# thodson-usgs/discontinuum

Hardware: AMD Instinct MI355X
Metric: GP fits/sec (NLL+grad step) at n=8192 d=3, 1/2/4/8 MI355X (higher is better)
Workload: dtype f64

## Files before the change

discontinuum_amd/_lib.py:

```python
from __future__ import annotations

import ctypes as C
import os

_HERE = os.path.dirname(os.path.abspath(__file__))
LIB_PATH = os.path.join(_HERE, "libdgp_hip.so")

F64, F32 = 0, 1
MODEL_LOADEST, MODEL_RATING = 0, 1
OUT_NLL, OUT_QUAD, OUT_LOGDET, OUT_INFO, OUT_DTHETA, OUT_SUM_DR, OUT_DR_W0, OUT_SUM_DNOISE, OUT_LEN = 0, 1, 2, 3, 4, 28, 29, 31, 32
BUF_XT, BUF_A, BUF_T, BUF_S, BUF_Z, BUF_ALPHA = range(6)
BUF_INFO, BUF_SCAL = 6, 7
OPT_LAUUM64_MAX_TILES, OPT_SYRK_SLOTS, OPT_TRTRI_SMALL, OPT_REFINE, OPT_SYRK_ORDER, OPT_LAUUM_ORDER, OPT_CHAIN_YIELD, OPT_FUSED_GRAD, OPT_GROUP_GEMM = range(9)
OPT_POTRF_SCHEDULE, OPT_POTRF_SWEEP, OPT_POTRF_SOLVE, OPT_POTRF_OVERLAP, OPT_POTRF_SLOTS, OPT_POTRF_TAIL, OPT_POTRF_TAIL_SWEEP = range(9, 16)
TIME_GRAM, TIME_POTRF, TIME_SYRK_SUM, TIME_SYRK_N, TIME_TRTRI, TIME_LAUUM, TIME_SOLVE, TIME_GRAD, TIME_SYRK_FLOP, TIME_COUNT = range(10)


E_ARG, E_MODEL, E_WORKSPACE, E_STATE, E_FULL, E_NOCONV = -1, -2, -3, -4, -5, -6


class DGPLibraryError(RuntimeError):
    pass


class DGPError(RuntimeError):
    def __init__(self, code, where, msg):
        super().__init__(f"{where} failed with code {code}: {msg}")
        self.code = code


_vp, _i, _i64, _sz = C.c_void_p, C.c_int, C.c_int64, C.c_size_t
_dp = C.POINTER(C.c_double)

SIGNATURES = {
    "dgp_version": (_i, []),
    "dgp_last_error": (C.c_char_p, []),
    "dgp_model_ntheta": (_i, [_i, _i]),
# ... 124 lines not shown
```

discontinuum_amd/csrc/dgp_api.hip:

```cpp
#include <mutex>
#include <new>
#include <stdio.h>
#include <stdlib.h>
#include <string.h>
#include <utility>
#include <vector>

#include "../../include/dgp_hip.h"
#include "dgp_common.h"
#include "dgp_internal.h"

using namespace dgp;

static thread_local char g_err[256] = "";
static int fail(int code, const char* msg) {
  snprintf(g_err, sizeof(g_err), "%s", msg);
  return code;
}
static int hipfail(hipError_t e, const char* where) {
  snprintf(g_err, sizeof(g_err), "%s: %s", where, hipGetErrorString(e));
  return (int)e;
}

struct PinnedRing {
// ... 30 lines not shown
      if (have_ev[i]) (void)hipEventDestroy(ev[i]);
      if (buf[i]) (void)hipHostFree(buf[i]);
    }
  }
};

struct dgp_plan {
  int model, dtype, d, ntheta;
  PinnedRing ring;
  int* nsite_host;
  int B;
  size_t site_bytes;
  void* pre;
  void* pre2;
  int pre_ready;
  Tuning tune;
  int refine;
  int* nsite;
  const void* dr_w;
  int64_t n, N;
  size_t elem;
  char* ws;
  size_t ws_bytes;
  void *Xt, *A, *Tm, *S, *z, *alpha, *gpart, *spart, *scal, *snap;
  int* info;
  hipStream_t sc;
  int lookahead, early;
  int have_inputs, have_factor, have_inverse;
  hipStream_t s2, s3;
  hipEvent_t xev[8];
  int have_xev;
  hipEvent_t* ev;
  int nev;
  int timing, n_syrk, timed_valid;
  double syrk_flop;
  hipEvent_t* tev;
  hipEvent_t* sev;
  int nsev;
};
enum { TS_GRAM = 0, TS_POTRF, TS_TRTRI, TS_LAUUM, TS_SOLVE, TS_GRAD, TS_COUNT };

static size_t align_up(size_t x) { return (x + 255) & ~(size_t)255; }

struct Layout {
  size_t Xt, A, Tm, S, z, alpha, gpart, spart, scal, info, snap, total;
};
static Layout layout(const dgp_plan* p) {
  Layout L;
  const size_t e = p->elem, N = (size_t)p->N;
  size_t o = 0;
  L.Xt = o; o += align_up(e * N * p->d);
  L.A = o; o += align_up(e * N * N);
  L.Tm = o; o += align_up(e * N * N);
  L.S = o; o += align_up(e * N * N);
  L.z = o; o += align_up(e * N);
  L.alpha = o; o += align_up(e * N);
  L.gpart = o; o += align_up(e * (size_t)gram_grad_partials(p->N));
  L.spart = o; o += align_up(e * (size_t)solve_partials(p->N));
  L.scal = o; o += align_up(e * 16);
  L.info = o; o += align_up(sizeof(int) * POTRF_INFO_INTS);
  L.snap = o; o += align_up(e * 2 * DGP_TILE_HOST * DGP_TILE_HOST);
  L.total = o;
  return L;
}

static int default_lookahead() { return 2; }
static int group_size(int lookahead, int batch, long nbk) {
  if (!lookahead) return 0;
  if (const char* e = getenv("DGP_GROUP")) return atoi(e) < 2 ? 2 : atoi(e);
  if (batch >= 4) return 4;
  return nbk >= 256 ? 8 : (nbk >= 96 ? 4 : 2);
}

#define EARLY_WG_CAP 384
#define EARLY_RESERVED_CUS 64

extern "C" {

int dgp_version(void) { return 1; }
const char* dgp_last_error(void) { return g_err; }
int dgp_model_ntheta(int model, int d) { return model_ntheta(model, d); }
int dgp_composite_define(const int* spec, int nspec, int* model_out) {
  if (!spec || nspec < 2 || !model_out) return fail(DGP_E_ARG, "dgp_composite_define: null argument");
  const int id = composite_define(spec, nspec);
// ... 89 lines not shown
  return 0;
}

int dgp_plan_set_workspace(dgp_plan* p, void* dev_ptr, size_t bytes) {
  if (!p || !dev_ptr) return fail(DGP_E_ARG, "dgp_plan_set_workspace: null");
  const Layout L = layout(p);
  if (bytes < dgp_plan_workspace_bytes(p))
    return fail(DGP_E_WORKSPACE, "dgp_plan_set_workspace: workspace too small");
  p->site_bytes = L.total;
  if (((uintptr_t)dev_ptr & 255) != 0) return fail(DGP_E_ARG, "dgp_plan_set_workspace: pointer must be 256-byte aligned");
  p->ws = (char*)dev_ptr;
  p->ws_bytes = bytes;
  p->Xt = p->ws + L.Xt;
  p->A = p->ws + L.A;
  p->Tm = p->ws + L.Tm;
  p->S = p->ws + L.S;
  p->z = p->ws + L.z;
  p->alpha = p->ws + L.alpha;
  p->gpart = p->ws + L.gpart;
  p->spart = p->ws + L.spart;
  p->scal = p->ws + L.scal;
  p->info = (int*)(p->ws + L.info);
  p->snap = p->ws + L.snap;
  p->pre = pre_scratch_bytes(p->B) ? (void*)(p->ws + L.total * (size_t)p->B) : nullptr;
  p->pre2 = p->pre ? (void*)((char*)p->pre + align_up(pre_scratch_bytes(p->B))) : nullptr;
  p->nsite = nullptr;
  p->dr_w = nullptr;
  if (p->B > 1) {
    p->nsite = (int*)(p->ws + L.total * (size_t)p->B + 2 * align_up(pre_scratch_bytes(p->B)));
    delete[] p->nsite_host;
    p->nsite_host = new (std::nothrow) int[(size_t)p->B];
    if (!p->nsite_host) return fail(DGP_E_ARG, "dgp_plan_set_workspace: out of host memory");
    for (int b = 0; b < p->B; ++b) p->nsite_host[b] = (int)p->n;
    hipError_t e = hipMemcpy(p->nsite, p->nsite_host, sizeof(int) * (size_t)p->B, hipMemcpyHostToDevice);
    if (e != hipSuccess) return hipfail(e, "dgp_plan_set_workspace: hipMemcpy");
  }
  p->have_inputs = p->have_factor = 0;
  return 0;
}

int dgp_plan_set_option(dgp_plan* p, int key, int64_t value) {
  if (!p) return fail(DGP_E_ARG, "dgp_plan_set_option: null plan");
  switch (key) {
    case DGP_OPT_LAUUM64_MAX_TILES:
      if (value < 0 || value > (1 << 30)) return fail(DGP_E_ARG, "dgp_plan_set_option: value out of range");
      p->tune.lauum64_max_tiles = (int)value;
// ... 20 lines not shown
    case DGP_OPT_GROUP_GEMM:
      p->tune.group_gemm = value ? 1 : 0;
      return 0;
    case DGP_OPT_POTRF_SCHEDULE:
      if (value < 0 || value > 1) return fail(DGP_E_ARG, "dgp_plan_set_option: value out of range");
      p->tune.potrf_schedule = (int)value;
      return 0;
    case DGP_OPT_POTRF_SWEEP:
    case DGP_OPT_POTRF_TAIL:
    case DGP_OPT_POTRF_TAIL_SWEEP:
      if (value < 0 || value > (1 << 20)) return fail(DGP_E_ARG, "dgp_plan_set_option: value out of range");
      (key == DGP_OPT_POTRF_SWEEP ? p->tune.potrf_sweep : key == DGP_OPT_POTRF_TAIL ? p->tune.potrf_tail : p->tune.potrf_tail_sweep) = (int)value;
      return 0;
    case DGP_OPT_POTRF_SOLVE:
      p->tune.potrf_solve = value ? 1 : 0;
      return 0;
    case DGP_OPT_POTRF_OVERLAP:
      p->tune.potrf_overlap = value ? 1 : 0;
      return 0;
    case DGP_OPT_POTRF_SLOTS:
      if (value < 1 || value > (1 << 20)) return fail(DGP_E_ARG, "dgp_plan_set_option: value out of range");
      p->tune.potrf_slots = (int)value;
      return 0;
    case DGP_OPT_REFINE:
      if (p->dtype != DGP_F32 && value) return fail(DGP_E_ARG, "dgp_plan_set_option: refinement applies to float32 plans");
      p->refine = value ? 1 : 0;
      return 0;
    default:
      return fail(DGP_E_ARG, "dgp_plan_set_option: unknown option");
  }
}
int dgp_plan_get_option(const dgp_plan* p, int key, int64_t* value) {
  if (!p || !value) return fail(DGP_E_ARG, "dgp_plan_get_option: null argument");
  switch (key) {
    case DGP_OPT_LAUUM64_MAX_TILES: *value = p->tune.lauum64_max_tiles; return 0;
    case DGP_OPT_SYRK_SLOTS: *value = p->tune.syrk_slots; return 0;
    case DGP_OPT_TRTRI_SMALL: *value = p->tune.trtri_small; return 0;
    case DGP_OPT_REFINE: *value = p->refine; return 0;
    case DGP_OPT_SYRK_ORDER: *value = p->tune.syrk_super; return 0;
    case DGP_OPT_LAUUM_ORDER: *value = p->tune.lauum_super; return 0;
    case DGP_OPT_CHAIN_YIELD: *value = p->tune.chain_yield; return 0;
    case DGP_OPT_FUSED_GRAD: *value = p->tune.fused_grad; return 0;
    case DGP_OPT_GROUP_GEMM: *value = p->tune.group_gemm; return 0;
    case DGP_OPT_POTRF_SCHEDULE:
      *value = p->tune.potrf_schedule < 0 ? (p->B >= 4 ? potrf_schedule_auto(p->B, p->N / DGP_TILE_HOST, p->elem) : 0) : p->tune.potrf_schedule;
      return 0;
    case DGP_OPT_POTRF_SWEEP: *value = p->tune.potrf_sweep; return 0;
    case DGP_OPT_POTRF_SOLVE: *value = p->tune.potrf_solve; return 0;
    case DGP_OPT_POTRF_OVERLAP: *value = p->tune.potrf_overlap; return 0;
    case DGP_OPT_POTRF_SLOTS: *value = p->tune.potrf_slots; return 0;
    case DGP_OPT_POTRF_TAIL: *value = p->tune.potrf_tail; return 0;
    case DGP_OPT_POTRF_TAIL_SWEEP: *value = p->tune.potrf_tail_sweep; return 0;
    default: return fail(DGP_E_ARG, "dgp_plan_get_option: unknown option");
  }
}

int dgp_plan_set_lookahead(dgp_plan* p, int level) {
  if (!p) return fail(DGP_E_ARG, "null plan");
  p->lookahead = level ? default_lookahead() : 0;
  p->early = level >= 2 && !getenv("DGP_NO_EARLY_TRTRI");
  return 0;
}

size_t dgp_plan_site_stride_bytes(const dgp_plan* p) { return p ? layout(p).total : 0; }

int dgp_plan_buffer(const dgp_plan* p, int which, void** dev_ptr, int64_t* ld) {
  if (!p || !dev_ptr || !p->ws) return fail(DGP_E_ARG, "dgp_plan_buffer: null / no workspace");
  void* q = nullptr;
  switch (which) {
    case DGP_BUF_XT: q = p->Xt; break;
    case DGP_BUF_A: q = p->A; break;
    case DGP_BUF_T: q = p->Tm; break;
    case DGP_BUF_S: q = p->S; break;
    case DGP_BUF_Z: q = p->z; break;
    case DGP_BUF_ALPHA: q = p->alpha; break;
// ... 268 lines not shown
    const long N = p->N;
    const size_t nb = (size_t)(N / 64), part_bytes = nb * nb * 64 * sizeof(double);
    if (gram_residual_scratch_bytes(N) > (size_t)N * N * sizeof(float)) return 0;
    char* base = (char*)p->S;
    double* part = (double*)base;
    double* rho64 = (double*)(base + part_bytes);
    float* rho32 = (float*)(base + part_bytes + (size_t)N * sizeof(double));
    float* delta = rho32 + N;
    const Batch bt = batch_of<float>(p);
    const long ps = bt.ws / 2;
    void* staging = p->pre2 ? p->ring.acquire(pre_scratch_bytes(p->B)) : nullptr;
    int rc = gram_residual<float>(p->model, p->d, (const float*)p->Xt, N, (int)p->n, theta, (const float*)noise, (const float*)r,
                                  (const float*)p->alpha, part, rho64, rho32, s, bt, ps, bt.ws, p->pre2, staging);
    if (staging) p->ring.commit(s);
    if (rc) return rc;
    return refine_solve<float>((const float*)p->Tm, N, (const float*)r, (int)p->n, rho64, rho32, (float*)p->z, delta,
                               (float*)p->alpha, (float*)p->spart, (float*)p->scal + 1, s, bt, ps, bt.ws);
  }
}

template <typename T>
static int run_grad(dgp_plan* p, const double* theta, void* dtheta, hipStream_t s) {
  return gram_grad<T>(p->model, p->d, (const T*)p->Xt, p->N, (int)p->n, theta, (const T*)p->S, (const T*)p->alpha,
                      (T*)p->gpart, (T*)dtheta, s, batch_of<T>(p), DGP_OUT_LEN, p->pre, p->pre_ready != 0);
}

template <typename T>
static bool solve_overlap(const dgp_plan* p) {
  if (p->N < 1024 || p->N > 6144 || !p->lookahead || !p->ev || p->nev < 2 || !p->s2) return false;
  return !(sizeof(T) == 4 && p->refine);
}

template <typename T>
static int fit_step(dgp_plan* p, const double* theta, const void* r, const void* noise, void* out, void* dr,
                    void* dnoise, int with_grad, hipStream_t s) {
  int rc;
  if ((rc = ensure_timing(p))) return rc;
  tick(p, TS_GRAM, 0, s);
  if ((rc = run_gram<T>(p, theta, noise, s))) return rc;
  tick(p, TS_GRAM, 1, s);
  if ((rc = ensure_async(p, s)) || (rc = ensure_early(p, s))) return rc;
  tick(p, TS_POTRF, 0, s);
  const int nbk = (int)(p->N / DGP_TILE_HOST);
  const bool early = early_applies(p) && p->s3 != nullptr;
  const Batch bt = batch_of<T>(p);
  if (early) {
    struct Early {
// ... 1164 lines not shown
```

discontinuum_amd/csrc/dgp_chol.hip:

```cpp
#include <stdlib.h>
#include <string.h>
#include <algorithm>
#include <mutex>
#include "dgp_diag.h"
#include "dgp_gemm.h"
#include "dgp_gemm_dma.h"
#include "dgp_internal.h"
#include "dgp_schedule.h"

namespace dgp {

static constexpr int NB = DGP_TILE;
static constexpr int SMID_TABLE = 4096;
template <typename T>
struct Prefetch {
  static constexpr bool F64 = sizeof(T) == 8;
  static constexpr int LAUUM = F64 ? 2 : 4, TRTRI = F64 ? 1 : 4, SYRK = F64 ? 1 : 2;
};

#define DGP_INFO_CHAIN_TIMEOUT (-7)
#define CHAIN_WAIT_TICKS 200000000LL
__device__ __forceinline__ bool chain_reached(const int* word, int value) {
  return __hip_atomic_load(word, __ATOMIC_RELAXED, __HIP_MEMORY_SCOPE_AGENT) >= value;
}
// ... 101 lines not shown
  if (super > 0) super_decode(nfull + sub / split, nt, super, bi, bj);
  else tri_decode(nfull + sub / split, bi, bj);
  syrk_cut_tile<T>(A, ld, k, nk, (long)(bi + jbeg) * NB, (long)(bj + jbeg) * NB, split, sub % split, smem);
}

const Tuning& default_tuning() {
  static const Tuning t = [] {
    Tuning v;
    v.lauum64_max_tiles = getenv("DGP_LAUUM64") ? atoi(getenv("DGP_LAUUM64")) : 1000;
    v.syrk_slots = getenv("DGP_SYRK_SLOTS") ? atoi(getenv("DGP_SYRK_SLOTS")) : 512;
    v.trtri_small = getenv("DGP_TRTRI_SMALL") ? atol(getenv("DGP_TRTRI_SMALL")) : 1024;
    v.syrk_super = getenv("DGP_SYRK_ORDER") ? atoi(getenv("DGP_SYRK_ORDER")) : 0;
    v.lauum_super = getenv("DGP_LAUUM_ORDER") ? atoi(getenv("DGP_LAUUM_ORDER")) : 0;
    v.chain_yield = getenv("DGP_CHAIN_YIELD") ? atoi(getenv("DGP_CHAIN_YIELD")) : 1;
    v.fused_grad = getenv("DGP_FUSED_GRAD") ? atoi(getenv("DGP_FUSED_GRAD")) : 0;
    v.group_gemm = getenv("DGP_GROUP_GEMM") ? atoi(getenv("DGP_GROUP_GEMM")) : 0;
    v.potrf_schedule = getenv("DGP_POTRF_SCHEDULE") ? (atoi(getenv("DGP_POTRF_SCHEDULE")) != 0 ? 1 : 0) : -1;
    v.potrf_sweep = getenv("DGP_POTRF_SWEEP") ? std::max(0, atoi(getenv("DGP_POTRF_SWEEP"))) : 0;
    v.potrf_tail = getenv("DGP_POTRF_TAIL") ? std::max(0, atoi(getenv("DGP_POTRF_TAIL"))) : 0;
    v.potrf_tail_sweep = getenv("DGP_POTRF_TAIL_SWEEP") ? std::max(0, atoi(getenv("DGP_POTRF_TAIL_SWEEP"))) : 0;
    v.potrf_solve = getenv("DGP_POTRF_SOLVE") ? atoi(getenv("DGP_POTRF_SOLVE")) : 0;
    v.potrf_overlap = getenv("DGP_POTRF_OVERLAP") ? atoi(getenv("DGP_POTRF_OVERLAP")) : 0;
    v.potrf_slots = getenv("DGP_POTRF_SLOTS") ? std::max(1, atoi(getenv("DGP_POTRF_SLOTS"))) : 768;
    if (v.syrk_slots < 1) v.syrk_slots = 1;
    return v;
  }();
  return t;
}
int potrf_schedule_auto(int B, long nbk, int elem) { return (elem == 8 && B >= 32 && nbk > 4) ? 1 : 0; }
struct SyrkShape {
  int nfull, split;
  unsigned grid;
  explicit SyrkShape(int ntiles, int slots = 512) {
    if (slots < 1) slots = 1;
    const double cost[5] = {0, 1.0, 0.55, 0, 0.30};
    const int whole = ntiles / slots * slots, rem = ntiles - whole;
    nfull = ntiles;
    split = 1;
    double best = (ntiles + slots - 1) / slots * cost[1];
    for (int g = 2; g <= 4; g += 2) {
      const double c = whole / slots * cost[1] + (g * rem + slots - 1) / slots * cost[g];
      if (rem > 0 && c < best - 1e-9) {
        best = c;
        nfull = whole;
        split = g;
      }
// ... 1153 lines not shown
```

discontinuum_amd/csrc/dgp_gram.hip:

```cpp
#include <mutex>
#include <string.h>
#include "dgp_internal.h"
#include "dgp_models.h"
#include "dgp_gram_shared.h"

namespace dgp {

size_t pre_scratch_bytes(int B) { return B > DGP_MAX_BATCH ? (size_t)B * DGP_PRE_SLOT_BYTES : 0; }

#define DGP_C_MAXMODELS 64
static CompositeDesc g_comp[DGP_C_MAXMODELS];
static int g_ncomp = 0;
static std::mutex g_comp_mtx;
static thread_local const CompositeDesc* g_comp_cur = nullptr;
const CompositeDesc* composite_current() { return g_comp_cur; }
static const CompositeDesc* composite_get(int model) {
  const int slot = model - DGP_MODEL_COMPOSITE_BASE;
  return (slot >= 0 && slot < g_ncomp) ? &g_comp[slot] : nullptr;
}
bool composite_select(int model, int d) {
  g_comp_cur = composite_get(model);
  return g_comp_cur && g_comp_cur->d == d;
}

// ... 27 lines not shown
      fc.ls = (signed char)th;
      th += ard ? ndims : 1;
      fc.period = type == DGP_FAC_PERIODIC ? (signed char)th++ : (signed char)-1;
      if (th > DGP_MAX_THETA) return -2;
    }
  }
  if (i != nspec) return -2;
  c.ntheta = (unsigned char)th;
  std::lock_guard<std::mutex> lock(g_comp_mtx);
  for (int k = 0; k < g_ncomp; ++k)
    if (memcmp(&g_comp[k], &c, sizeof(c)) == 0) return DGP_MODEL_COMPOSITE_BASE + k;
  if (g_ncomp >= DGP_C_MAXMODELS) return -5;
  g_comp[g_ncomp] = c;
  return DGP_MODEL_COMPOSITE_BASE + g_ncomp++;
}

int model_ntheta(int model, int d) {
  if (model == DGP_MODEL_LOADEST) return (d >= 2 && d <= 6) ? 2 * d + 5 : -1;
  if (model == DGP_MODEL_RATING) return d == 2 ? 16 : -1;
  if (const CompositeDesc* c = composite_get(model)) return c->d == d ? c->ntheta : -1;
  return -1;
}

int model_nterms(int model, int d) {
  if (model == DGP_MODEL_LOADEST) return (d >= 2 && d <= 6) ? 3 : -1;
  if (model == DGP_MODEL_RATING) return d == 2 ? 5 : -1;
  if (const CompositeDesc* c = composite_get(model)) return c->d == d ? c->nterms : -1;
  return -1;
}

int model_input_differentiable(int model, int d, int col) {
  if (model_ntheta(model, d) < 0 || col < 0 || col >= d) return -1;
  const CompositeDesc* c = composite_get(model);
  if (!c) return 1;
  for (int t = 0; t < c->nterms; ++t)
    for (int f = 0; f < c->term[t].nfac; ++f) {
      const CompositeDesc::Fac& fc = c->term[t].fac[f];
      if (fc.type != DGP_FAC_MATERN || fc.nu2 != 1) continue;
      for (int j = 0; j < fc.ndims; ++j)
        if (fc.dims[j] == col) return 0;
    }
  return 1;
}

template <typename T>
__global__ __launch_bounds__(256) void pack_x_kernel(const T* __restrict__ X, int n, int d, long N, T* __restrict__ Xt,
// ... 93 lines not shown
      if (gi >= n || gj >= m) v = T(0);
      out[b] = v;
    }
    store4<T>(Ks + gi * Mp + (long)bj * 64 + tx * 4, out);
  }
}

template <typename T, typename M>
__global__ __launch_bounds__(256) void gram_diag_kernel(const T* __restrict__ Xst, long Mp, int m, const PreBatch<M> pb,
                                                        T* __restrict__ kss, long wbs) {
  const typename M::Pre& pre = pb.get();
  Xst = site(Xst, wbs);
  kss = site(kss, wbs);
  exp_table_init<T>();
  __syncthreads();
  const long j = (long)blockIdx.x * 256 + threadIdx.x;
  if (j >= Mp) return;
  T x[M::NX], f[M::NF], dummy[M::NTHETA];
#pragma unroll
  for (int c = 0; c < M::NX; ++c) x[c] = Xst[(long)c * Mp + j];
  M::features(x, pre, f);
  T v = M::template pair<false>(f, f, pre, T(0), dummy);
  kss[j] = j < m ? v : T(0);
}

template <typename T, typename M, int MODE>
__global__ __launch_bounds__(256) void gram_grad_kernel(const T* __restrict__ Xt, long N, int n, const PreBatch<M> pb,
                                                        const T* __restrict__ S, const T* __restrict__ alpha,
                                                        const T* __restrict__ beta, T* __restrict__ partials, long bs,
                                                        const int* __restrict__ ns, long wbs ) {
  n = site_n(ns, n);
  const typename M::Pre& pre = pb.get();
  Xt = site(Xt, bs);
  if (MODE == 0) S = site(S, bs);
  alpha = site(alpha, bs);
  partials = site(partials, MODE == 0 ? bs : wbs);
  if (MODE == 1) beta = site(beta, wbs);
  __shared__ T sfi[M::NF][64], sfj[M::NF][64], sai[64], saj[64], sbi[64], sbj[64];
  __shared__ T red[4][M::NTHETA];
  int bi, bj;
  tri_decode(blockIdx.x, bi, bj);
  const int t = threadIdx.x;
  exp_table_init<T>();
  if (t < 64) {
    stage_strip<T, M>(Xt, N, (long)bi * 64, pre, sfi, t);
    sai[t] = alpha[(long)bi * 64 + t];
// ... 311 lines not shown
  const int nb = (int)(N / 64);
  const double* p = part + (i / 64) * (long)nb * 64 + (i & 63);
  double s0 = 0.0, s1 = 0.0, s2 = 0.0, s3 = 0.0;
  int b = 0;
  for (; b + 4 <= nb; b += 4) {
    s0 += p[(long)b * 64];
    s1 += p[(long)(b + 1) * 64];
    s2 += p[(long)(b + 2) * 64];
    s3 += p[(long)(b + 3) * 64];
  }
  for (; b < nb; ++b) s0 += p[(long)b * 64];
  double v = 0.0;
  if (i < n) v = (double)r[i] - (double)noise[i] * (double)alpha[i] - ((s0 + s1) + (s2 + s3));
  rho64[i] = v;
  rho32[i] = (TS)v;
}

template <typename T>
int pack_x(const T* X, int n, int d, long N, T* Xt, hipStream_t s, Batch bt) {
  pack_x_kernel<T><<<dim3((unsigned)((N + 255) / 256), 1, (unsigned)bt.B), dim3(256), 0, s>>>(X, n, d, N, Xt, bt.ws, bt.ns);
  return (int)hipGetLastError();
}

template <typename T>
int gram_sym(int model, int d, const T* Xt, long N, int n, const double* theta, const T* noise, T* K, hipStream_t s,
             Batch bt, void* pre_scratch, void* pre_staging, long k_stride, long noise_stride, bool pre_ready) {
  const int nt = model_ntheta(model, d);
  if (nt < 0) return -2;
  const long nb = N / 64;
  const unsigned grid = (unsigned)(nb * (nb + 1) / 2);
  const long ks = k_stride >= 0 ? k_stride : bt.ws, nstr = noise_stride >= 0 ? noise_stride : (long)n;
  DGP_DISPATCH_MODEL(model, d, (gram_sym_kernel<T, M><<<dim3(grid, 1, (unsigned)bt.B), dim3(256), 0, s>>>(
                                   Xt, N, n, prepare_batch<M>(theta, nt, bt.B, pre_scratch, !pre_ready, s, pre_staging), noise, K, bt.ws, bt.ns,
                                   ks, nstr)));
  return (int)hipGetLastError();
}

template <typename T>
int gram_sym_panel(int model, int d, const T* Xt, long N, int n, const double* theta, const T* noise, T* K, long row0, long row1,
                   hipStream_t s, Batch bt, void* pre_scratch, long k_stride, long noise_stride) {
  const int nt = model_ntheta(model, d);
  if (nt < 0) return -2;
  const long b0 = row0 / 64, b1 = row1 / 64;
  const long t0 = b0 * (b0 + 1) / 2, t1 = b1 * (b1 + 1) / 2;
  DGP_DISPATCH_MODEL(model, d, (gram_sym_kernel<T, M, true><<<dim3((unsigned)(t1 - t0), 1, (unsigned)bt.B), dim3(256), 0, s>>>(
                                   Xt, N, n, prepare_batch<M>(theta, nt, bt.B, pre_scratch, false, s), noise, K, bt.ws, bt.ns, k_stride,
// ... 11 lines not shown
                                   Xt, N, n, Xst, Mp, m, prepare_batch<M>(theta, nt, bt.B, pre_scratch, true, s, pre_staging), Ks, bt.ws,
                                   wbs, bt.ns)));
  return (int)hipGetLastError();
}

template <typename T>
int gram_diag(int model, int d, const T* Xst, long Mp, int m, const double* theta, T* kss, hipStream_t s, Batch bt, long wbs,
              void* pre_scratch) {
  const int nt = model_ntheta(model, d);
  if (nt < 0) return -2;
  dim3 grid((unsigned)((Mp + 255) / 256), 1, (unsigned)bt.B);
  DGP_DISPATCH_MODEL(model, d, (gram_diag_kernel<T, M><<<grid, dim3(256), 0, s>>>(
                                   Xst, Mp, m, prepare_batch<M>(theta, nt, bt.B, pre_scratch, false, s), kss, wbs)));
  return (int)hipGetLastError();
}

long gram_grad_partials(long N) {
  const long nb = N / 64;
  return nb * (nb + 1) / 2 * DGP_MAX_THETA;
}

template <typename T>
int gram_grad(int model, int d, const T* Xt, long N, int n, const double* theta, const T* S, const T* alpha,
              T* partials, T* dtheta, hipStream_t s, Batch bt, long dtheta_stride, void* pre_scratch, bool pre_ready,
              void* pre_staging) {
  const int nt = model_ntheta(model, d);
  if (nt < 0) return -2;
  const long nb = N / 64;
  const long nblk = nb * (nb + 1) / 2;
  DGP_DISPATCH_MODEL(model, d,
                     (gram_grad_kernel<T, M, 0><<<dim3((unsigned)nblk, 1, (unsigned)bt.B), dim3(256), 0, s>>>(
                         Xt, N, n, prepare_batch<M>(theta, nt, bt.B, pre_scratch, !pre_ready, s, pre_staging), S, alpha, nullptr,
                         partials, bt.ws, bt.ns, 0)));
  grad_reduce_kernel<T><<<dim3((unsigned)nt, 1, (unsigned)bt.B), dim3(256), 0, s>>>(partials, nblk, nt, dtheta, 0, bt.ws,
                                                                                 dtheta_stride);
  return (int)hipGetLastError();
}

template <typename T>
int mean_vjp_grad(int model, int d, const T* Xt, long N, int n, const T* Xst, long Mp, int m, const double* theta,
                  const T* alpha, const T* beta, const T* wts, T* partials, T* dtheta, hipStream_t s, Batch bt, long wbs,
                  long dstride, void* pre_scratch, void* pre_staging) {
  const int nt = model_ntheta(model, d);
  if (nt < 0) return -2;
  const long nb = N / 64;
  const long nblk = nb * (nb + 1) / 2;
  const unsigned Bz = (unsigned)bt.B;
  DGP_DISPATCH_MODEL(model, d,
                     (gram_grad_kernel<T, M, 1><<<dim3((unsigned)nblk, 1, Bz), dim3(256), 0, s>>>(
                         Xt, N, n, prepare_batch<M>(theta, nt, bt.B, pre_scratch, true, s, pre_staging), nullptr, alpha, beta, partials,
                         bt.ws, bt.ns, wbs)));
  grad_reduce_kernel<T><<<dim3((unsigned)nt, 1, Bz), dim3(256), 0, s>>>(partials, nblk, nt, dtheta, 0, wbs, dstride);
  dim3 grid((unsigned)(Mp / 64), (unsigned)(N / 64), Bz);
  DGP_DISPATCH_MODEL(model, d,
                     (gram_cross_grad_kernel<T, M><<<grid, dim3(256), 0, s>>>(
                         Xt, N, n, Xst, Mp, m, prepare_batch<M>(theta, nt, bt.B, pre_scratch, false, s), alpha, wts, partials, bt.ws, wbs,
                         bt.ns)));
// ... 40 lines not shown
                  const TS* alpha, double* part, double* rho64, TS* rho32, hipStream_t s, Batch bt, long ps, long rs,
                  void* pre_scratch, void* pre_staging) {
  using T = double;
  const int nt = model_ntheta(model, d);
  if (nt < 0) return -2;
  const long nb = N / 64;
  const unsigned grid = (unsigned)(nb * (nb + 1) / 2);
  DGP_DISPATCH_MODEL(model, d, (gram_matvec_kernel<TS, M><<<dim3(grid, 1, (unsigned)bt.B), dim3(256), 0, s>>>(
                                   Xt, N, n, prepare_batch<M>(theta, nt, bt.B, pre_scratch, true, s, pre_staging), alpha, part, bt.ws, ps,
                                   bt.ns)));
  resid_reduce_kernel<TS><<<dim3((unsigned)((N + 255) / 256), 1, (unsigned)bt.B), dim3(256), 0, s>>>(part, N, n, r, noise, alpha, rho64,
                                                                                                 rho32, bt.ws, ps, rs, bt.ns);
  return (int)hipGetLastError();
}
template int gram_residual<float>(int, int, const float*, long, int, const double*, const float*, const float*, const float*,
                                  double*, double*, float*, hipStream_t, Batch, long, long, void*, void*);

#define DGP_INST(T)                                                                                              \
  template int pack_x<T>(const T*, int, int, long, T*, hipStream_t, Batch);                                      \
  template int gram_sym<T>(int, int, const T*, long, int, const double*, const T*, T*, hipStream_t, Batch, void*, void*, long, long, bool); \
  template int gram_sym_panel<T>(int, int, const T*, long, int, const double*, const T*, T*, long, long, hipStream_t, Batch, void*, long, long); \
  template int gram_cross<T>(int, int, const T*, long, int, const T*, long, int, const double*, T*, hipStream_t, Batch, long, void*, void*); \
  template int gram_diag<T>(int, int, const T*, long, int, const double*, T*, hipStream_t, Batch, long, void*);    \
  template int gram_grad<T>(int, int, const T*, long, int, const double*, const T*, const T*, T*, T*, hipStream_t, Batch, \
                            long, void*, bool, void*);                                                         \
  template int mean_vjp_grad<T>(int, int, const T*, long, int, const T*, long, int, const double*, const T*, const T*, \
                                const T*, T*, T*, hipStream_t, Batch, long, long, void*, void*);                    \
  template int gemv_rows<T>(const T*, long, long, int, const T*, T*, hipStream_t, int, long);                   \
  template int gram_slab<T>(int, int, const T*, long, int, const double*, const T*, T*, long, SlabMap, hipStream_t); \
  template int gram_grad_slab<T>(int, int, const T*, long, int, const double*, const T*, long, SlabMap, const T*, T*, T*, T*, \
                                 hipStream_t);
DGP_INST(double)
DGP_INST(float)

}
```

discontinuum_amd/csrc/dgp_internal.h:

```cpp
#pragma once
#include <hip/hip_runtime.h>
#include <stdint.h>

#define DGP_TILE_HOST 128

namespace dgp {

inline long round_up(long n, long q) { return (n + q - 1) / q * q; }

#define DGP_MAX_BATCH_HOST 8
#define DGP_MAX_BATCH_SITES 1024
struct Tuning {
  int lauum64_max_tiles;
  int syrk_slots;
  long trtri_small;
  int syrk_super;
  int lauum_super;
  int chain_yield;
  int fused_grad;
  int group_gemm;
  int potrf_schedule;
  int potrf_sweep;
  int potrf_tail;
  int potrf_tail_sweep;
  int potrf_solve;
  int potrf_slots;
  int potrf_overlap;
};
const Tuning& default_tuning();
int potrf_schedule_auto(int B, long nbk, int elem);
struct Batch {
  int B = 1;
  long ws = 0;
  const int* ns = nullptr;
  const Tuning* tune = nullptr;
  void* W = nullptr;
  const Tuning& tuning() const { return tune ? *tune : default_tuning(); }
};
int model_ntheta(int model, int d);
int model_nterms(int model, int d);
int composite_define(const int* spec, int nspec);
bool composite_select(int model, int d);

template <typename T>
int pack_x(const T* X, int n, int d, long N, T* Xt, hipStream_t s, Batch bt = Batch());
template <typename T>
int gram_sym(int model, int d, const T* Xt, long N, int n, const double* theta, const T* noise, T* K, hipStream_t s,
             Batch bt = Batch(), void* pre_scratch = nullptr ,
             void* pre_staging = nullptr ,
             long k_stride = -1 , long noise_stride = -1 ,
             bool pre_ready = false );
template <typename T>
int gram_sym_panel(int model, int d, const T* Xt, long N, int n, const double* theta, const T* noise, T* K, long row0, long row1,
                   hipStream_t s, Batch bt, void* pre_scratch, long k_stride, long noise_stride);
template <typename T>
int gram_cross(int model, int d, const T* Xt, long N, int n, const T* Xst, long M, int m, const double* theta,
               T* Ks, hipStream_t s, Batch bt = Batch(), long wbs = 0, void* pre_scratch = nullptr, void* pre_staging = nullptr);
template <typename T>
int gram_diag(int model, int d, const T* Xst, long M, int m, const double* theta, T* kss, hipStream_t s, Batch bt = Batch(),
              long wbs = 0, void* pre_scratch = nullptr);
template <typename T>
int gram_grad(int model, int d, const T* Xt, long N, int n, const double* theta, const T* S, const T* alpha,
              T* partials, T* dtheta, hipStream_t s, Batch bt = Batch(), long dtheta_stride = 0,
              void* pre_scratch = nullptr, bool pre_ready = false ,
              void* pre_staging = nullptr);
size_t pre_scratch_bytes(int B);
template <typename TS>
int gram_residual(int model, int d, const TS* Xt, long N, int n, const double* theta, const TS* noise, const TS* r,
                  const TS* alpha, double* part, double* rho64, TS* rho32, hipStream_t s, Batch bt, long ps, long rs,
                  void* pre_scratch, void* pre_staging);
size_t gram_residual_scratch_bytes(long N);
long gram_grad_partials(long N);
bool lauum_grad_applies(int model, long N, const Batch& bt);
template <typename T>
int lauum_grad(int model, int d, const T* Tm, long N, T* S, const T* Xt, int n, const double* theta, const T* alpha, T* partials,
               T* dtheta, hipStream_t s, Batch bt, long dtheta_stride, void* pre_scratch, bool pre_ready, void* pre_staging);
template <typename T>
int mean_vjp_grad(int model, int d, const T* Xt, long N, int n, const T* Xst, long Mp, int m, const double* theta,
                  const T* alpha, const T* beta, const T* wts, T* partials, T* dtheta, hipStream_t s, Batch bt = Batch(),
                  long wbs = 0, long dstride = 0, void* pre_scratch = nullptr, void* pre_staging = nullptr);
template <typename T>
int gemv_rows(const T* Ks, long N, long Mp, int m, const T* w, T* out, hipStream_t s, int B = 1, long wbs = 0);

struct PotrfObservers {
  hipEvent_t* syrk_ev = nullptr;
  int syrk_pool = 0;
// ... 264 lines not shown
```

include/dgp_hip.h:

```cpp
#ifndef DGP_HIP_H
#define DGP_HIP_H
#include <stddef.h>
#include <stdint.h>

#ifdef __cplusplus
extern "C" {
#endif

#define DGP_F64 0
#define DGP_F32 1
#define DGP_MODEL_LOADEST 0
#define DGP_MODEL_RATING 1

#define DGP_E_ARG (-1)
#define DGP_E_MODEL (-2)
#define DGP_E_WORKSPACE (-3)
#define DGP_E_STATE (-4)
#define DGP_E_FULL (-5)
#define DGP_E_NOCONV (-6)

#define DGP_OUT_NLL 0
#define DGP_OUT_QUAD 1
#define DGP_OUT_LOGDET 2
#define DGP_OUT_INFO 3
// ... 25 lines not shown
size_t dgp_plan_workspace_bytes(const dgp_plan* plan);
int dgp_plan_set_batch(dgp_plan* plan, int batch);
int dgp_plan_batch(const dgp_plan* plan);
int dgp_plan_set_site_sizes(dgp_plan* plan, const int64_t* sizes_host, void* stream);
int dgp_plan_set_workspace(dgp_plan* plan, void* dev_ptr, size_t bytes);
int dgp_plan_set_dr_weights(dgp_plan* plan, const void* w_dev);
int dgp_plan_set_lookahead(dgp_plan* plan, int level);
#define DGP_OPT_LAUUM64_MAX_TILES 0
#define DGP_OPT_SYRK_SLOTS 1
#define DGP_OPT_TRTRI_SMALL 2
#define DGP_OPT_REFINE 3
#define DGP_OPT_SYRK_ORDER 4
#define DGP_OPT_LAUUM_ORDER 5
#define DGP_OPT_CHAIN_YIELD 6
#define DGP_OPT_FUSED_GRAD 7
#define DGP_OPT_GROUP_GEMM 8
#define DGP_OPT_POTRF_SCHEDULE 9
#define DGP_OPT_POTRF_SWEEP 10
#define DGP_OPT_POTRF_SOLVE 11
#define DGP_OPT_POTRF_OVERLAP 12
#define DGP_OPT_POTRF_SLOTS 13
#define DGP_OPT_POTRF_TAIL 14
#define DGP_OPT_POTRF_TAIL_SWEEP 15
int dgp_plan_set_option(dgp_plan* plan, int key, int64_t value);
int dgp_plan_get_option(const dgp_plan* plan, int key, int64_t* value_out);
int dgp_plan_buffer(const dgp_plan* plan, int which, void** dev_ptr, int64_t* ld);
size_t dgp_plan_site_stride_bytes(const dgp_plan* plan);

int dgp_set_inputs(dgp_plan* plan, const void* X_dev, void* stream);

int dgp_fit_step(dgp_plan* plan, const double* theta_host, const void* r_dev, const void* noise_dev,
                 void* out_dev, void* dr_dev, void* dnoise_dev, void* stream);

int dgp_factorize(dgp_plan* plan, const double* theta_host, const void* r_dev, const void* noise_dev,
                  void* out_dev, void* stream);

size_t dgp_laplace_workspace_bytes(const dgp_plan* plan);
int dgp_laplace_fit_step(dgp_plan* plan, const double* theta_host, const void* y_dev, const void* mean_dev, const void* noise_dev,
                         const int32_t* side_dev, void* f_dev, int maxit, double tol, void* work_dev, size_t work_bytes,
                         void* out_dev, void* dr_dev, double* stat_host, void* stream);
int dgp_laplace_factorize(dgp_plan* plan, const double* theta_host, const void* y_dev, const void* mean_dev, const void* noise_dev,
                          const int32_t* side_dev, void* f_dev, int maxit, double tol, void* work_dev, size_t work_bytes,
                          void* out_dev, double* stat_host, void* stream);
size_t dgp_laplace_batched_workspace_bytes(const dgp_plan* plan);
int dgp_laplace_batched_fit_step(dgp_plan* plan, const double* theta_host, const void* y_dev, const void* mean_dev,
                                 const void* noise_dev, const int32_t* side_dev, void* f_dev, int maxit, double tol, void* work_dev,
// ... 149 lines not shown
```

Measured before the change: 116.9.

## Precompute features and process gradient tiles in row runs for reuse

Adds a kernel that writes each point's model features to a workspace buffer once. The gradient kernel is replaced by one where each block walks a run of R adjacent column tiles in the same row, reusing the row strip's features and double-buffering the column strips in shared memory. This cuts redundant feature computation and the number of partial sums to reduce. It costs extra workspace and a feature pass, and lowers parallelism when runs are long. It is enabled by default only for the f64 Loadest d=3 model, with the run length chosen by a heuristic.

```diff
diff --git a/discontinuum_amd/_lib.py b/discontinuum_amd/_lib.py
--- a/discontinuum_amd/_lib.py
+++ b/discontinuum_amd/_lib.py
@@ -13,6 +13,7 @@
 BUF_INFO, BUF_SCAL = 6, 7
 OPT_LAUUM64_MAX_TILES, OPT_SYRK_SLOTS, OPT_TRTRI_SMALL, OPT_REFINE, OPT_SYRK_ORDER, OPT_LAUUM_ORDER, OPT_CHAIN_YIELD, OPT_FUSED_GRAD, OPT_GROUP_GEMM = range(9)
 OPT_POTRF_SCHEDULE, OPT_POTRF_SWEEP, OPT_POTRF_SOLVE, OPT_POTRF_OVERLAP, OPT_POTRF_SLOTS, OPT_POTRF_TAIL, OPT_POTRF_TAIL_SWEEP = range(9, 16)
+OPT_GRAM_RUN = 16
 TIME_GRAM, TIME_POTRF, TIME_SYRK_SUM, TIME_SYRK_N, TIME_TRTRI, TIME_LAUUM, TIME_SOLVE, TIME_GRAD, TIME_SYRK_FLOP, TIME_COUNT = range(10)
 
 
diff --git a/discontinuum_amd/csrc/dgp_api.hip b/discontinuum_amd/csrc/dgp_api.hip
--- a/discontinuum_amd/csrc/dgp_api.hip
+++ b/discontinuum_amd/csrc/dgp_api.hip
@@ -76,7 +76,7 @@
   size_t elem;
   char* ws;
   size_t ws_bytes;
-  void *Xt, *A, *Tm, *S, *z, *alpha, *gpart, *spart, *scal, *snap;
+  void *Xt, *A, *Tm, *S, *z, *alpha, *gpart, *spart, *scal, *snap, *feat;
   int* info;
   hipStream_t sc;
   int lookahead, early;
@@ -97,7 +97,7 @@
 static size_t align_up(size_t x) { return (x + 255) & ~(size_t)255; }
 
 struct Layout {
-  size_t Xt, A, Tm, S, z, alpha, gpart, spart, scal, info, snap, total;
+  size_t Xt, A, Tm, S, z, alpha, gpart, spart, scal, info, snap, feat, total;
 };
 static Layout layout(const dgp_plan* p) {
   Layout L;
@@ -114,6 +114,7 @@
   L.scal = o; o += align_up(e * 16);
   L.info = o; o += align_up(sizeof(int) * POTRF_INFO_INTS);
   L.snap = o; o += align_up(e * 2 * DGP_TILE_HOST * DGP_TILE_HOST);
+  L.feat = o; o += align_up(e * N * (size_t)model_nfeat(p->model, p->d));
   L.total = o;
   return L;
 }
@@ -249,6 +250,7 @@
   p->scal = p->ws + L.scal;
   p->info = (int*)(p->ws + L.info);
   p->snap = p->ws + L.snap;
+  p->feat = p->ws + L.feat;
   p->pre = pre_scratch_bytes(p->B) ? (void*)(p->ws + L.total * (size_t)p->B) : nullptr;
   p->pre2 = p->pre ? (void*)((char*)p->pre + align_up(pre_scratch_bytes(p->B))) : nullptr;
   p->nsite = nullptr;
@@ -315,6 +317,10 @@
       if (value < 1 || value > (1 << 20)) return fail(DGP_E_ARG, "dgp_plan_set_option: value out of range");
       p->tune.potrf_slots = (int)value;
       return 0;
+    case DGP_OPT_GRAM_RUN:
+      if (value < 0 || value > 64) return fail(DGP_E_ARG, "dgp_plan_set_option: value out of range");
+      p->tune.gram_run = (int)value;
+      return 0;
     case DGP_OPT_REFINE:
       if (p->dtype != DGP_F32 && value) return fail(DGP_E_ARG, "dgp_plan_set_option: refinement applies to float32 plans");
       p->refine = value ? 1 : 0;
@@ -344,6 +350,7 @@
     case DGP_OPT_POTRF_SLOTS: *value = p->tune.potrf_slots; return 0;
     case DGP_OPT_POTRF_TAIL: *value = p->tune.potrf_tail; return 0;
     case DGP_OPT_POTRF_TAIL_SWEEP: *value = p->tune.potrf_tail_sweep; return 0;
+    case DGP_OPT_GRAM_RUN: *value = p->tune.gram_run; return 0;
     default: return fail(DGP_E_ARG, "dgp_plan_get_option: unknown option");
   }
 }
@@ -658,7 +665,7 @@
 template <typename T>
 static int run_grad(dgp_plan* p, const double* theta, void* dtheta, hipStream_t s) {
   return gram_grad<T>(p->model, p->d, (const T*)p->Xt, p->N, (int)p->n, theta, (const T*)p->S, (const T*)p->alpha,
-                      (T*)p->gpart, (T*)dtheta, s, batch_of<T>(p), DGP_OUT_LEN, p->pre, p->pre_ready != 0);
+                      (T*)p->gpart, (T*)p->feat, (T*)dtheta, s, batch_of<T>(p), DGP_OUT_LEN, p->pre, p->pre_ready != 0);
 }
 
 template <typename T>
diff --git a/discontinuum_amd/csrc/dgp_chol.hip b/discontinuum_amd/csrc/dgp_chol.hip
--- a/discontinuum_amd/csrc/dgp_chol.hip
+++ b/discontinuum_amd/csrc/dgp_chol.hip
@@ -147,6 +147,7 @@
     v.potrf_solve = getenv("DGP_POTRF_SOLVE") ? atoi(getenv("DGP_POTRF_SOLVE")) : 0;
     v.potrf_overlap = getenv("DGP_POTRF_OVERLAP") ? atoi(getenv("DGP_POTRF_OVERLAP")) : 0;
     v.potrf_slots = getenv("DGP_POTRF_SLOTS") ? std::max(1, atoi(getenv("DGP_POTRF_SLOTS"))) : 768;
+    v.gram_run = getenv("DGP_GRAM_RUN") ? std::min(64, std::max(0, atoi(getenv("DGP_GRAM_RUN")))) : 0;
     if (v.syrk_slots < 1) v.syrk_slots = 1;
     return v;
   }();
diff --git a/discontinuum_amd/csrc/dgp_gram.hip b/discontinuum_amd/csrc/dgp_gram.hip
--- a/discontinuum_amd/csrc/dgp_gram.hip
+++ b/discontinuum_amd/csrc/dgp_gram.hip
@@ -73,6 +73,13 @@
   return -1;
 }
 
+int model_nfeat(int model, int d) {
+  if (model == DGP_MODEL_LOADEST) return (d >= 2 && d <= 6) ? d + 2 : -1;
+  if (model == DGP_MODEL_RATING) return d == 2 ? 5 : -1;
+  if (const CompositeDesc* c = composite_get(model)) return c->d == d ? d : -1;
+  return -1;
+}
+
 int model_nterms(int model, int d) {
   if (model == DGP_MODEL_LOADEST) return (d >= 2 && d <= 6) ? 3 : -1;
   if (model == DGP_MODEL_RATING) return d == 2 ? 5 : -1;
@@ -212,6 +219,141 @@
   M::features(x, pre, f);
   T v = M::template pair<false>(f, f, pre, T(0), dummy);
   kss[j] = j < m ? v : T(0);
+}
+
+template <typename T, typename M>
+__global__ __launch_bounds__(256) void gram_features_kernel(const T* __restrict__ Xt, long N, const PreBatch<M> pb,
+                                                            T* __restrict__ feat, long bs) {
+  const typename M::Pre& pre = pb.get();
+  Xt = site(Xt, bs);
+  feat = site(feat, bs);
+  const long i = (long)blockIdx.x * 256 + threadIdx.x;
+  if (i >= N) return;
+  T x[M::NX], f[M::NF];
+#pragma unroll
+  for (int c = 0; c < M::NX; ++c) x[c] = Xt[(long)c * N + i];
+  M::features(x, pre, f);
+#pragma unroll
+  for (int c = 0; c < M::NF; ++c) feat[(long)c * N + i] = f[c];
+}
+
+template <typename T, int NF>
+__device__ __forceinline__ void strip_fetch(const T* __restrict__ feat, long N, long base, int t, T (&v)[(NF * 64 + 255) / 256]) {
+#pragma unroll
+  for (int q = 0; q < (NF * 64 + 255) / 256; ++q) {
+    const int idx = t + 256 * q;
+    if (idx < NF * 64) v[q] = feat[(long)(idx >> 6) * N + base + (idx & 63)];
+  }
+}
+template <typename T, int NF>
+__device__ __forceinline__ void strip_put(T (*sf)[64], int t, const T (&v)[(NF * 64 + 255) / 256]) {
+#pragma unroll
+  for (int q = 0; q < (NF * 64 + 255) / 256; ++q) {
+    const int idx = t + 256 * q;
+    if (idx < NF * 64) sf[idx >> 6][idx & 63] = v[q];
+  }
+}
+
+static long tri_runs(long nb, int R) {
+  const long k = nb / R, m = nb % R;
+  return R * k * (k + 1) / 2 + m * (k + 1);
+}
+__device__ __forceinline__ void run_decode(int idx, int R, int& bi, int& b0) {
+  int k = (int)((sqrtf(8.0f * (float)idx / (float)R + 1.0f) - 1.0f) * 0.5f);
+  while ((long)R * (k + 1) * (k + 2) / 2 <= idx) ++k;
+  while ((long)R * k * (k + 1) / 2 > idx) --k;
+  const int rem = idx - R * k * (k + 1) / 2;
+  bi = k * R + rem / (k + 1);
+  b0 = (rem % (k + 1)) * R;
+}
+static int gram_run_length(long nb, const Batch& bt) {
+  for (int R = 8; R > 1; R >>= 1)
+    if (nb >= 4 * R && tri_runs(nb, R) * bt.B >= 4096) return R;
+  return 1;
+}
+
+template <typename T, typename M, int WAVES>
+__global__ __launch_bounds__(256, WAVES) void gram_grad_rows_kernel(const T* __restrict__ feat, long N, int n, const PreBatch<M> pb,
+                                                             const T* __restrict__ S, const T* __restrict__ alpha,
+                                                             T* __restrict__ partials, long bs, const int* __restrict__ ns, int R) {
+  n = site_n(ns, n);
+  const typename M::Pre& pre = pb.get();
+  feat = site(feat, bs);
+  S = site(S, bs);
+  alpha = site(alpha, bs);
+  partials = site(partials, bs);
+  constexpr int NF = M::NF;
+  __shared__ T sfi[NF][64], sfj[2][NF][64], sai[64], saj[2][64];
+  __shared__ T red[4][M::NTHETA];
+  int bi, b0;
+  run_decode((int)blockIdx.x, R, bi, b0);
+  const int len = min(R, bi + 1 - b0);
+  const int t = threadIdx.x;
+  exp_table_init<T>();
+  T pf[(NF * 64 + 255) / 256];
+  strip_fetch<T, NF>(feat, N, (long)bi * 64, t, pf);
+  strip_put<T, NF>(sfi, t, pf);
+  strip_fetch<T, NF>(feat, N, (long)b0 * 64, t, pf);
+  strip_put<T, NF>(sfj[0], t, pf);
+  if (t < 64) sai[t] = alpha[(long)bi * 64 + t];
+  else if (t < 128) saj[0][t - 64] = alpha[(long)b0 * 64 + t - 64];
+  __syncthreads();
+  const int ty = t >> 4, tx = t & 15;
+  T acc[M::NTHETA];
+#pragma unroll
+  for (int p = 0; p < M::NTHETA; ++p) acc[p] = T(0);
+  const T* Srow = S + ((long)bi * 64 + ty * 4) * N + (long)b0 * 64 + tx * 4;
+  constexpr bool AHEAD = WAVES == 1;
+  T sv[4], nx[4] = {T(0), T(0), T(0), T(0)};
+  if (AHEAD) load4<T>(Srow, sv);
+  const bool rows_full = bi * 64 + 64 <= n;
+#pragma unroll 1
+  for (int k = 0; k < len; ++k) {
+    const int bj = b0 + k, cur = k & 1;
+    const bool more = k + 1 < len;
+    const bool diag = bj == bi, interior = !diag && rows_full;
+#pragma unroll 1
+    for (int a = 0; a < 4; ++a) {
+      if (!AHEAD) load4<T>(Srow + (long)a * N + k * 64, sv);
+      else if (a < 3) load4<T>(Srow + (long)(a + 1) * N + k * 64, nx);
+      else if (more) load4<T>(Srow + (k + 1) * 64, nx);
+      const int ri = ty * 4 + a;
+      T fi[NF];
+#pragma unroll
+      for (int c = 0; c < NF; ++c) fi[c] = sfi[c][ri];
+      const T ai = sai[ri];
+#pragma unroll 1
+      for (int b = 0; b < 4; ++b) {
+        const int cj = tx * 4 + b;
+        T fj[NF];
+#pragma unroll
+        for (int c = 0; c < NF; ++c) fj[c] = sfj[cur][c][cj];
+        const T svb = b == 0 ? sv[0] : (b == 1 ? sv[1] : (b == 2 ? sv[2] : sv[3]));
+        T w = svb - ai * saj[cur][cj];
+        if (!interior) w = ((diag && cj > ri) || bi * 64 + ri >= n) ? T(0) : ((diag && cj == ri) ? T(0.5) * w : w);
+        (void)M::template pair<true>(fi, fj, pre, w, acc);
+      }
+      if (AHEAD) {
+#pragma unroll
+        for (int q = 0; q < 4; ++q) sv[q] = nx[q];
+      }
+    }
+    if (more) {
+      strip_fetch<T, NF>(feat, N, (long)(bj + 1) * 64, t, pf);
+      strip_put<T, NF>(sfj[cur ^ 1], t, pf);
+      if (t < 64) saj[cur ^ 1][t] = alpha[(long)(bj + 1) * 64 + t];
+      __syncthreads();
+    }
+  }
+  M::finalize(acc, pre);
+  const int lane = t & 63, wv = t >> 6;
+#pragma unroll
+  for (int p = 0; p < M::NTHETA; ++p) {
+    T v = wave_sum(acc[p]);
+    if (lane == 0) red[wv][p] = v;
+  }
+  __syncthreads();
+  if (t < M::NTHETA) partials[(long)blockIdx.x * DGP_MAX_THETA + t] = red[0][t] + red[1][t] + red[2][t] + red[3][t];
 }
 
 template <typename T, typename M, int MODE>
@@ -569,6 +711,32 @@
   return (int)hipGetLastError();
 }
 
+template <typename T, typename M>
+struct RowsGrad { static constexpr bool pays = false; static constexpr int waves = 1; };
+template <>
+struct RowsGrad<double, Loadest<double, 3>> { static constexpr bool pays = true; static constexpr int waves = 4; };
+
+template <typename T, typename M>
+static void launch_grad(const T* Xt, long N, int n, const PreBatch<M>& pb, const T* S, const T* alpha, T* partials, T* feat, int R,
+                        hipStream_t s, const Batch& bt) {
+  const unsigned Bz = (unsigned)bt.B;
+  const long nb = N / 64;
+  if (R <= 1) {
+    gram_grad_kernel<T, M, 0><<<dim3((unsigned)(nb * (nb + 1) / 2), 1, Bz), dim3(256), 0, s>>>(Xt, N, n, pb, S, alpha, nullptr, partials,
+                                                                                         bt.ws, bt.ns, 0);
+    return;
+  }
+  gram_features_kernel<T, M><<<dim3((unsigned)((N + 255) / 256), 1, Bz), dim3(256), 0, s>>>(Xt, N, pb, feat, bt.ws);
+  gram_grad_rows_kernel<T, M, RowsGrad<T, M>::waves><<<dim3((unsigned)tri_runs(nb, R), 1, Bz), dim3(256), 0, s>>>(feat, N, n, pb, S, alpha,
+                                                                                                             partials, bt.ws, bt.ns, R);
+}
+template <typename T, typename M>
+static int grad_run_length(long nb, const Batch& bt, const T* feat) {
+  if (feat == nullptr) return 1;
+  if (bt.tuning().gram_run > 0) return bt.tuning().gram_run;
+  return RowsGrad<T, M>::pays ? gram_run_length(nb, bt) : 1;
+}
+
 template <typename T>
 int gram_sym(int model, int d, const T* Xt, long N, int n, const double* theta, const T* noise, T* K, hipStream_t s,
              Batch bt, void* pre_scratch, void* pre_staging, long k_stride, long noise_stride, bool pre_ready) {
@@ -626,17 +794,16 @@
 
 template <typename T>
 int gram_grad(int model, int d, const T* Xt, long N, int n, const double* theta, const T* S, const T* alpha,
-              T* partials, T* dtheta, hipStream_t s, Batch bt, long dtheta_stride, void* pre_scratch, bool pre_ready,
+              T* partials, T* feat, T* dtheta, hipStream_t s, Batch bt, long dtheta_stride, void* pre_scratch, bool pre_ready,
               void* pre_staging) {
   const int nt = model_ntheta(model, d);
   if (nt < 0) return -2;
-  const long nb = N / 64;
-  const long nblk = nb * (nb + 1) / 2;
-  DGP_DISPATCH_MODEL(model, d,
-                     (gram_grad_kernel<T, M, 0><<<dim3((unsigned)nblk, 1, (unsigned)bt.B), dim3(256), 0, s>>>(
-                         Xt, N, n, prepare_batch<M>(theta, nt, bt.B, pre_scratch, !pre_ready, s, pre_staging), S, alpha, nullptr,
-                         partials, bt.ws, bt.ns, 0)));
-  grad_reduce_kernel<T><<<dim3((unsigned)nt, 1, (unsigned)bt.B), dim3(256), 0, s>>>(partials, nblk, nt, dtheta, 0, bt.ws,
+  int R = 1;
+  DGP_DISPATCH_MODEL(model, d, (R = grad_run_length<T, M>(N / 64, bt, feat)));
+  const long nruns = tri_runs(N / 64, R);
+  DGP_DISPATCH_MODEL(model, d, (launch_grad<T, M>(Xt, N, n, prepare_batch<M>(theta, nt, bt.B, pre_scratch, !pre_ready, s, pre_staging), S,
+                                                  alpha, partials, feat, R, s, bt)));
+  grad_reduce_kernel<T><<<dim3((unsigned)nt, 1, (unsigned)bt.B), dim3(256), 0, s>>>(partials, nruns, nt, dtheta, 0, bt.ws,
                                                                                  dtheta_stride);
   return (int)hipGetLastError();
 }
@@ -723,7 +890,7 @@
   template int gram_sym_panel<T>(int, int, const T*, long, int, const double*, const T*, T*, long, long, hipStream_t, Batch, void*, long, long); \
   template int gram_cross<T>(int, int, const T*, long, int, const T*, long, int, const double*, T*, hipStream_t, Batch, long, void*, void*); \
   template int gram_diag<T>(int, int, const T*, long, int, const double*, T*, hipStream_t, Batch, long, void*);    \
-  template int gram_grad<T>(int, int, const T*, long, int, const double*, const T*, const T*, T*, T*, hipStream_t, Batch, \
+  template int gram_grad<T>(int, int, const T*, long, int, const double*, const T*, const T*, T*, T*, T*, hipStream_t, Batch, \
                             long, void*, bool, void*);                                                         \
   template int mean_vjp_grad<T>(int, int, const T*, long, int, const T*, long, int, const double*, const T*, const T*, \
                                 const T*, T*, T*, hipStream_t, Batch, long, long, void*, void*);                    \
diff --git a/discontinuum_amd/csrc/dgp_internal.h b/discontinuum_amd/csrc/dgp_internal.h
--- a/discontinuum_amd/csrc/dgp_internal.h
+++ b/discontinuum_amd/csrc/dgp_internal.h
@@ -26,6 +26,7 @@
   int potrf_solve;
   int potrf_slots;
   int potrf_overlap;
+  int gram_run;
 };
 const Tuning& default_tuning();
 int potrf_schedule_auto(int B, long nbk, int elem);
@@ -39,6 +40,7 @@
 };
 int model_ntheta(int model, int d);
 int model_nterms(int model, int d);
+int model_nfeat(int model, int d);
 int composite_define(const int* spec, int nspec);
 bool composite_select(int model, int d);
 
@@ -61,7 +63,8 @@
               long wbs = 0, void* pre_scratch = nullptr);
 template <typename T>
 int gram_grad(int model, int d, const T* Xt, long N, int n, const double* theta, const T* S, const T* alpha,
-              T* partials, T* dtheta, hipStream_t s, Batch bt = Batch(), long dtheta_stride = 0,
+              T* partials, T* feat , T* dtheta, hipStream_t s,
+              Batch bt = Batch(), long dtheta_stride = 0,
               void* pre_scratch = nullptr, bool pre_ready = false ,
               void* pre_staging = nullptr);
 size_t pre_scratch_bytes(int B);
diff --git a/include/dgp_hip.h b/include/dgp_hip.h
--- a/include/dgp_hip.h
+++ b/include/dgp_hip.h
@@ -71,6 +71,7 @@
 #define DGP_OPT_POTRF_SLOTS 13
 #define DGP_OPT_POTRF_TAIL 14
 #define DGP_OPT_POTRF_TAIL_SWEEP 15
+#define DGP_OPT_GRAM_RUN 16
 int dgp_plan_set_option(dgp_plan* plan, int key, int64_t value);
 int dgp_plan_get_option(const dgp_plan* plan, int key, int64_t* value_out);
 int dgp_plan_buffer(const dgp_plan* plan, int which, void** dev_ptr, int64_t* ld);
```

After: 117.2 (median of 6 runs). No clear change (+0.2%).
